# ai-forever/Kandinsky-2

Hardware: NVIDIA H100
Metric: unet_denoising_steps_per_sec (higher is better)
Workload: dtype f16

## Files before the change

include/k2b200.h:

```cpp
#ifndef K2B200_H_
#define K2B200_H_

#include <stdint.h>

#ifdef __cplusplus
extern "C" {
#endif

typedef void* k2_stream_t;

const char* k2_last_error(void);
int k2_version(void);
long long k2_launch_count(void);
void k2_reset_launch_count(void);
int k2_set_tuning(int key, int value);

typedef struct {
  const void* ptr;
  int C;
  int ld;
  int taps;
} K2ConvSrc;

int k2_conv_gemm(const K2ConvSrc* srcs, int nsrc, int NB, int H, int W, const void* w_packed, int w_rows,
                 int Ktot, int ldw, int Cout, const float* bias, const void* residual, int ldr, void* out, int ldo,
                 int out_mode, void* workspace, long long workspace_bytes, float* gn_partial, int* info,
                 k2_stream_t stream);

int k2_conv_gemm_cfg(const K2ConvSrc* srcs, int nsrc, int NB, int H, int W, const void* w_packed, int w_rows,
                     int Ktot, int ldw, int Cout, const float* bias, const void* residual, int ldr, void* out, int ldo,
                     int out_mode, void* workspace, long long workspace_bytes, float* gn_partial, int* info,
                     const int* cfg, long long w_batch_stride, k2_stream_t stream);

int k2_conv_plan(int NB, int H, int W, int taps, int Ktot, int Cout, int out_mode, long long workspace_bytes,
                 int want_gn_partial, int* info);

long long k2_gn_scratch_floats(int NB, int HW, int C);
int k2_gn_stats(const void* src0, int C0, int ld0, const void* src1, int C1, int ld1, int NB, int HW,
                int groups, float eps, float* stats, float* scratch, k2_stream_t stream);
int k2_gn_finalize(const float* part0, int C0, int rg0, const float* part1, int C1, int rg1, int NB, int HW, int groups,
                   float eps, float* stats, k2_stream_t stream);
int k2_gn_apply(const void* src0, int C0, int ld0, const void* src1, int C1, int ld1, int NB, int H, int W,
                int groups, const float* stats, const float* gamma, const float* beta, const float* film,
                int film_ld, int act, int resample, void* y, int ldy, void* xres, int ldx, const float* zq, int zh,
                int zw, const float* sn_w, k2_stream_t stream);
int k2_gn_apply_fold(const void* src0, int C0, int ld0, const void* src1, int C1, int ld1, int NB, int H, int W, int groups,
                     const float* part0, int rg0, const float* part1, int rg1, float eps, const float* gamma,
                     const float* beta, const float* film, int film_ld, int act, int resample, void* y, int ldy, void* xres,
                     int ldx, k2_stream_t stream);

int k2_attention_d64(const void* qkv, int ldq, int hs, int q_off, int k_off, int v_off, const void* enc,
                     int lde, int ehs, int ek_off, int ev_off, int B, int heads, int T, int Tc, float scale,
                     void* out, int ldo, k2_stream_t stream);

int k2_attention_d512(const void* qkv, int ldq, int q_off, int k_off, int v_off, int B, int T, float scale, void* out, int ldo,
                      k2_stream_t stream);

int k2_linear(const float* x, int ldx, const void* W, int w_is_half, const float* b, const float* add,
              int ldadd, float* y, int ldy, int M, int N, int K, int silu_in, int silu_out,
              k2_stream_t stream);
int k2_layernorm(const float* x, const float* gamma, const float* beta, float* y, int M, int N, float eps,
                 k2_stream_t stream);
int k2_timestep_embedding(const float* t, float* out, int B, int dim, float max_period, k2_stream_t stream);
int k2_f32_to_f16(const float* x, void* y, long long n, k2_stream_t stream);
int k2_silu_f16(const void* x, void* y, long long n, k2_stream_t stream);

int k2_stem_im2col(const float* x, int Cx, const float* x2, int C2, const float* x3, int C3, int mul23,
                   int NB, int H, int W, void* out, int Kpad, k2_stream_t stream);
// ... 92 lines not shown
```

kandinsky-2_b200/csrc/k2_api.cu:

```cuda
#include <stdio.h>
#include <stdlib.h>
#include <string.h>

#include <algorithm>
#include <atomic>
#include <mutex>

#include "../../include/k2b200.h"
#include "k2_internal.h"

namespace k2 {

static thread_local std::string g_err;
static std::atomic<long long> g_launches{0};
static int g_force_bn = 0;
static int g_force_split = 0;
static int g_pdl = 0;


void set_error(const std::string& msg) { g_err = msg; }
int fail(const std::string& msg) {
  g_err = msg;
  return -1;
}
void count_launch(int n) { g_launches.fetch_add(n, std::memory_order_relaxed); }

bool pdl_enabled() { return g_pdl != 0; }
static int g_gn_bps = 0;
int gn_apply_blocks_per_sm() { return g_gn_bps; }

int num_sms() {
  static int n = 0;
  if (n == 0) {
    int dev = 0;
    cudaGetDevice(&dev);
    cudaDeviceGetAttribute(&n, cudaDevAttrMultiProcessorCount, dev);
    if (n <= 0) n = 132;
  }
  return n;
}

typedef CUresult (*EncodeTiledFn)(CUtensorMap*, CUtensorMapDataType, cuuint32_t, void*, const cuuint64_t*,
                                  const cuuint64_t*, const cuuint32_t*, const cuuint32_t*,
                                  CUtensorMapInterleave, CUtensorMapSwizzle, CUtensorMapL2promotion,
                                  CUtensorMapFloatOOBfill);

static EncodeTiledFn get_encode_fn() {
  static EncodeTiledFn fn = nullptr;
  static std::once_flag once;
  std::call_once(once, [] {
// ... 49 lines not shown
      const long long tiles = tiles_h * tiles_w * ((NB + tn - 1) / tn);
      for (int k = (tn == 1 ? 0 : 1); k < 2; ++k) {
        bool better = best_tiles[k] < 0 || tiles < best_tiles[k];
        if (!better && tiles == best_tiles[k]) {
          if (tn != bn[k]) {
            better = tn < bn[k];
          } else {
            const int d_new = tw > th ? tw - th : th - tw;
            const int d_old = bw[k] > bh[k] ? bw[k] - bh[k] : bh[k] - bw[k];
            better = (d_new < d_old) || (d_new == d_old && tw > bw[k]);
          }
        }
        if (better) {
          best_tiles[k] = tiles;
          bn[k] = tn;
          bw[k] = tw;
          bh[k] = th;
        }
      }
    }
  }
  const int k = (!single_image_only && best_tiles[1] * 100 <= best_tiles[0] * 85) ? 1 : 0;
  TN = bn[k];
  TW = bw[k];
  TH = bh[k];
}


struct ConvPlan {
  int TN, TH, TW, tiles_w, tiles_h, tiles_n, m_tiles;
  int m_tiles_phase;
  int BN, splits;
  int fuse_stats, row_groups;
};

static void plan_conv(int NB, int H, int W, bool any9, int kchunks, int Cout, int out_mode, bool has_workspace,
                      long long workspace_bytes, bool want_gn, ConvPlan& pl, const int* cfg = nullptr, bool up2 = false,
                      bool w_batched = false) {
  const int g_force_bn = (cfg && cfg[0]) ? cfg[0] : k2::g_force_bn;
  const int g_force_split = (cfg && cfg[2]) ? cfg[2] : k2::g_force_split;
  choose_tile(NB, H, W, pl.TN, pl.TH, pl.TW, w_batched);
  pl.tiles_w = (W + pl.TW - 1) / pl.TW;
  pl.tiles_h = (H + pl.TH - 1) / pl.TH;
  pl.tiles_n = (NB + pl.TN - 1) / pl.TN;
  pl.m_tiles = pl.tiles_w * pl.tiles_h * pl.tiles_n;
  pl.m_tiles_phase = pl.m_tiles;

  int BN = g_force_bn;
  int splits = 1;
  const long long M_total = static_cast<long long>(NB) * H * W;
  const bool can_split = !up2 && !w_batched && has_workspace && out_mode == 0 && Cout % 8 == 0;
  auto split_ok = [&](int sp) {
    if (sp == 1) return true;
    const int kps = (kchunks + sp - 1) / sp;
    return can_split && kps >= 8 && (sp - 1) * kps < kchunks &&
           static_cast<long long>(sp) * M_total * Cout * 4 <= workspace_bytes;
  };
  auto model = [&](int bn, int sp) {
    const long long nt = (Cout + bn - 1) / bn;
    const long long units = static_cast<long long>(pl.m_tiles) * nt * sp * (up2 ? 4 : 1);
    const long long slots = num_sms();
    const long long waves = (units + slots - 1) / slots;
    const long long kps = (kchunks + sp - 1) / sp;
    long long cost = waves * (kps * (4LL * bn + 60) + 2000);
    if (sp > 1) cost += 4000 + (static_cast<long long>(sp) + 1) * M_total * Cout * 4 / 1800;
    return cost;
  };
  if (BN == 0) {
    if (Cout <= 16) BN = 16;
    else if (Cout <= 64) BN = 64;
    else if (Cout <= 128) BN = 128;
    else BN = 0;
  }
  {
    const int cand[3] = {256, 192, 128};
    long long best = -1;
    int best_bn = BN ? BN : 256, best_sp = 1;
    for (int ci = 0; ci < 3; ++ci) {
      const int bn = BN ? BN : cand[ci];
      if (BN && ci > 0) break;
      for (int sp = 1; sp <= 8; ++sp) {
        if (g_force_split > 0 && sp != g_force_split) continue;
        if (!split_ok(sp)) continue;
        const long long c = model(bn, sp);
        if (best < 0 || c < best) {
          best = c;
          best_bn = bn;
          best_sp = sp;
        }
      }
    }
    BN = best_bn;
    splits = best_sp;
  }
  pl.BN = BN;
  pl.splits = splits;

  pl.fuse_stats = 0;
  pl.row_groups = 0;
  if (want_gn && out_mode == 0 && Cout % 8 == 0) {
    if (splits == 1 && BN >= 64 && Cout % 64 == 0 && (pl.TN == 1 || pl.TH * pl.TW == 16)) {
      pl.fuse_stats = 1;
      pl.row_groups = ((pl.TN == 1) ? pl.m_tiles : NB * pl.tiles_h * pl.tiles_w) * (up2 ? 4 : 1);
    } else if (splits > 1 && (static_cast<long long>(H) * W) % 16 == 0) {
      pl.fuse_stats = 2;
      pl.row_groups = static_cast<int>(M_total / 16);
    }
  }
}

static void plan_to_info(const ConvPlan& pl, int* info) {
  if (!info) return;
  info[0] = pl.BN; info[1] = 0;
  info[2] = pl.splits; info[3] = pl.m_tiles; info[4] = pl.TN;
  info[5] = pl.fuse_stats; info[6] = pl.row_groups;
}

}

using namespace k2;

extern "C" {

const char* k2_last_error(void) { return g_err.c_str(); }
int k2_version(void) { return 100; }
long long k2_launch_count(void) { return g_launches.load(); }
void k2_reset_launch_count(void) { g_launches.store(0); }
int k2_set_tuning(int key, int value) {
  if (key == 0) {
    g_force_bn = value;
    return 0;
  }
  if (key == 1) {
    g_force_split = value;
    return 0;
  }
  if (key == 2) {
    if (value == 2) return fail("k2_set_tuning: no CTA-pair conv kernel on sm_90");
    return 0;
  }
  if (key == 4) {
    g_pdl = value;
    return 0;
  }
  if (key == 10) {
    return 0;
  }
  if (key == 11) {
    g_gn_bps = value;
    return 0;
  }
  if (key == 9) {
    return 0;
  }

  return fail("k2_set_tuning: unknown key");
}

int k2_conv_gemm(const K2ConvSrc* srcs, int nsrc, int NB, int H, int W, const void* w_packed, int w_rows,
                 int Ktot, int ldw, int Cout, const float* bias, const void* residual, int ldr, void* out, int ldo,
                 int out_mode, void* workspace, long long workspace_bytes, float* gn_partial, int* info,
                 k2_stream_t stream) {
  return k2_conv_gemm_cfg(srcs, nsrc, NB, H, W, w_packed, w_rows, Ktot, ldw, Cout, bias, residual, ldr, out, ldo, out_mode,
                          workspace, workspace_bytes, gn_partial, info, nullptr, 0, stream);
}

int k2_conv_gemm_cfg(const K2ConvSrc* srcs, int nsrc, int NB, int H, int W, const void* w_packed, int w_rows,
                     int Ktot, int ldw, int Cout, const float* bias, const void* residual, int ldr, void* out, int ldo,
                     int out_mode, void* workspace, long long workspace_bytes, float* gn_partial, int* info,
                     const int* cfg, long long w_batch_stride, k2_stream_t stream) {
  K2_REQUIRE(w_batch_stride >= 0 && w_batch_stride % 8 == 0, "conv_gemm_cfg: w_batch_stride must be a multiple of 8 elements");
  K2_REQUIRE(out_mode == 0 || out_mode == 1, "conv_gemm: out_mode must be 0 (fp16 rows) or 1 (fp32 NCHW)");
  K2_REQUIRE(out_mode == 0 || residual == nullptr, "conv_gemm: out_mode 1 (fp32 NCHW) takes no residual");
  const bool w_batched = w_batch_stride > 0;
  if (cfg) {
    K2_REQUIRE(cfg[0] == 0 || cfg[0] == 16 || cfg[0] == 64 || cfg[0] == 128 || cfg[0] == 192 || cfg[0] == 256,
               "conv_gemm_cfg: N tile must be 0, 16, 64, 128, 192 or 256");
    K2_REQUIRE(cfg[1] >= 0 && cfg[1] <= 2 && cfg[2] >= 0 && cfg[2] <= 8 && cfg[3] >= 0 && cfg[3] <= 2,
// ... 56 lines not shown
  p.up2 = up2 ? 1 : 0;
  p.a_box_bytes = static_cast<uint32_t>(p.TN * p.TH * p.TW * 128);
  for (int s = 0; s < nsrc; ++s) {
    const K2ConvSrc& src = srcs[s];
    uint64_t dims[4] = {static_cast<uint64_t>(src.C), static_cast<uint64_t>(W), static_cast<uint64_t>(H),
                        static_cast<uint64_t>(NB)};
    uint64_t str[3] = {static_cast<uint64_t>(src.ld) * 2, static_cast<uint64_t>(src.ld) * 2 * W,
                       static_cast<uint64_t>(src.ld) * 2 * W * H};
    uint32_t box[4] = {64, static_cast<uint32_t>(p.TW), static_cast<uint32_t>(p.TH), static_cast<uint32_t>(p.TN)};
    if (encode_tmap_f16(&p.tmA[s], src.ptr, 4, dims, str, box)) return -1;
  }
  const int BN = pl.BN, splits = pl.splits, fuse_stats = pl.fuse_stats;
  p.splits = splits;
  p.k_per_split = (kchunks + splits - 1) / splits;
  p.M_total = static_cast<long long>(NB) * H * W * (up2 ? 4 : 1);
  p.ws = reinterpret_cast<float*>(workspace);
  p.n_tiles = (Cout + BN - 1) / BN;
  p.Cout = Cout;
  {
    uint64_t dims[3] = {static_cast<uint64_t>(Ktot), static_cast<uint64_t>(w_rows), static_cast<uint64_t>(w_batched ? NB : 1)};
    uint64_t str[2] = {static_cast<uint64_t>(ldw) * 2,
                       (w_batched ? static_cast<uint64_t>(w_batch_stride) : static_cast<uint64_t>(ldw) * w_rows) * 2};
    uint32_t box[3] = {64, static_cast<uint32_t>(BN), 1};
    if (encode_tmap_f16(&p.tmB, w_packed, 3, dims, str, box)) return -1;
  }
  p.bias = bias;
  p.residual = reinterpret_cast<const __half*>(residual);
  p.ldr = ldr;
  p.out = out;
  p.ldo = ldo;
  p.out_mode = (splits > 1) ? 2 : out_mode;
  p.gn_part = (fuse_stats == 1) ? reinterpret_cast<float2*>(gn_partial) : nullptr;
  p.gn_mode = (fuse_stats == 1) ? (p.TN == 1 ? 1 : 2) : 0;
  if (out_mode == 0) {
    K2_REQUIRE(ldo % 8 == 0 && (reinterpret_cast<uintptr_t>(out) & 15) == 0, "conv_gemm: out alignment");
    if (residual)
      K2_REQUIRE(ldr % 8 == 0 && (reinterpret_cast<uintptr_t>(residual) & 15) == 0, "conv_gemm: residual alignment");
  }
  int rc = launch_conv_gemm(p, BN, static_cast<cudaStream_t>(stream));
  if (rc == 0) g_launches.fetch_add(1, std::memory_order_relaxed);
  if (rc == 0 && splits > 1) {
    rc = launch_splitk_finalize(p.ws, splits, p.M_total, Cout, bias, p.residual, ldr, reinterpret_cast<__half*>(out), ldo,
                                fuse_stats == 2 ? reinterpret_cast<float2*>(gn_partial) : nullptr,
                                static_cast<cudaStream_t>(stream));
    if (rc == 0) g_launches.fetch_add(1, std::memory_order_relaxed);
  }
  return rc;
}

int k2_conv_plan(int NB, int H, int W, int taps, int Ktot, int Cout, int out_mode, long long workspace_bytes,
                 int want_gn_partial, int* info) {
  K2_REQUIRE(NB > 0 && H > 0 && W > 0 && Cout > 0 && info, "conv_plan: bad arguments");
  K2_REQUIRE(Ktot > 0 && Ktot % 64 == 0, "conv_plan: Ktot must be a positive multiple of 64");
  ConvPlan pl;
  plan_conv(NB, H, W, taps == 9, Ktot / 64, Cout, out_mode, workspace_bytes > 0, workspace_bytes, want_gn_partial != 0, pl);
  plan_to_info(pl, info);
  return 0;
}

}
```

kandinsky-2_b200/csrc/k2_conv_gemm.cu:

```cuda
#include <stdio.h>

#include "k2_common.cuh"
#include "k2_internal.h"

namespace k2 {

namespace {

constexpr int BM = 128;
constexpr int BK = 64;
constexpr int A_STAGE_BYTES = BM * BK * 2;
constexpr int EPI_WARP_BYTES = 16 * 128;
constexpr int SMEM_LIMIT = 227 * 1024;

template <int BN>
struct Cfg {
  static constexpr int B_STAGE_BYTES = BN * BK * 2;
  static constexpr int STAGE_BYTES = A_STAGE_BYTES + B_STAGE_BYTES;
  static constexpr int EPI_BYTES = 8 * (EPI_WARP_BYTES + BN * 4);
  static constexpr int BAR_BYTES = 256;
  static constexpr int FIXED = EPI_BYTES + BAR_BYTES + 1024;
  static constexpr int STAGES = (SMEM_LIMIT - FIXED) / STAGE_BYTES > 6 ? 6 : (SMEM_LIMIT - FIXED) / STAGE_BYTES;
  static constexpr int SMEM_BYTES = STAGES * STAGE_BYTES + FIXED;
  static_assert(STAGES >= 2, "conv_gemm: shared memory does not hold two pipeline stages");
};

__device__ __forceinline__ void decode_m_tile(const ConvGemmParams& p, int m_idx, int& n0, int& y0,
                                              int& x0, int& phase) {
  phase = 0;
  if (p.up2) {
    phase = m_idx / p.m_tiles_phase;
    m_idx -= phase * p.m_tiles_phase;
  }
  int tw_i = m_idx % p.tiles_w;
  int t = m_idx / p.tiles_w;
  int th_i = t % p.tiles_h;
  int tn_i = t / p.tiles_h;
  x0 = tw_i * p.TW;
  y0 = th_i * p.TH;
  n0 = tn_i * p.TN;
}

__device__ __forceinline__ void ldsm_x4(uint32_t (&r)[4], uint32_t saddr) {
  asm volatile("ldmatrix.sync.aligned.m8n8.x4.shared.b16 {%0, %1, %2, %3}, [%4];"
               : "=r"(r[0]), "=r"(r[1]), "=r"(r[2]), "=r"(r[3])
               : "r"(saddr)
               : "memory");
}

template <int BN>
__device__ __forceinline__ void epilogue_warp(const ConvGemmParams& p, const float (&acc)[BN / 2], float* epi, uint32_t stg,
                                              const float* bsm, int k, int lane, int n0, int y0, int x0, int cbase, int split,
                                              int m_idx, int phase) {
  const int thw = p.TH * p.TW;
  auto out_row_of = [&](int row, int& n, int& y, int& x) -> long long {
    const int tn = row / thw;
    const int rem = row - tn * thw;
    const int th = rem / p.TW;
    const int tw = rem - th * p.TW;
    n = n0 + tn;
    y = y0 + th;
    x = x0 + tw;
    if (tn >= p.TN || n >= p.NB || y >= p.H || x >= p.W) return -1;
    return p.up2 ? (static_cast<long long>(n) * (2 * p.H) + (2 * y + (phase >> 1))) * (2 * p.W) + (2 * x + (phase & 1))
                 : (static_cast<long long>(n) * p.H + y) * p.W + x;
  };
  const int t4 = lane & 3, ra = lane >> 2;
  if constexpr (BN % 64 == 0) {
    if ((p.out_mode == 0 && p.Cout % 64 == 0) || (p.out_mode == 2 && p.Cout % 32 == 0)) {
      int n_, y_, x_;
      const int my_pix = static_cast<int>(out_row_of(16 * k + (lane & 15), n_, y_, x_));
      const int sub = lane >> 3, piece = lane & 7;
      int pix[4];
// ... 142 lines not shown
      return;
    }
  }
  int n[2], y[2], x[2];
  long long orow[2];
#pragma unroll
  for (int h = 0; h < 2; ++h) orow[h] = out_row_of(16 * k + ra + 8 * h, n[h], y[h], x[h]);
#pragma unroll
  for (int q = 0; q < BN / 8; ++q) {
#pragma unroll
    for (int h = 0; h < 2; ++h) {
#pragma unroll
      for (int e = 0; e < 2; ++e) {
        const int col = cbase + 8 * q + 2 * t4 + e;
        if (orow[h] < 0 || col >= p.Cout) continue;
        float f = acc[4 * q + 2 * h + e];
        if (p.out_mode == 2) {
          p.ws[(static_cast<long long>(split) * p.M_total + orow[h]) * p.Cout + col] = f;
          continue;
        }
        if (p.bias) f += __ldg(p.bias + col);
        if (p.out_mode == 0) {
          if (p.residual) f += __half2float(p.residual[orow[h] * p.ldr + col]);
          reinterpret_cast<__half*>(p.out)[orow[h] * p.ldo + col] = __float2half_rn(f);
        } else {
          reinterpret_cast<float*>(p.out)[((static_cast<long long>(n[h]) * p.Cout + col) * p.H + y[h]) * p.W + x[h]] = f;
        }
      }
    }
  }
}


template <int BN>
__global__ void __launch_bounds__(384, 1) conv_gemm_kernel(const __grid_constant__ ConvGemmParams p) {
  using C = Cfg<BN>;
  constexpr int NA = BN / 2;
  extern __shared__ uint8_t smem_raw[];
  uint8_t* smem = reinterpret_cast<uint8_t*>((reinterpret_cast<uintptr_t>(smem_raw) + 1023) &
                                             ~static_cast<uintptr_t>(1023));
  float* epi = reinterpret_cast<float*>(smem + C::STAGES * C::STAGE_BYTES);
  uint64_t* full_bar = reinterpret_cast<uint64_t*>(smem + C::STAGES * C::STAGE_BYTES + C::EPI_BYTES);
  uint64_t* empty_bar = full_bar + C::STAGES;

  const int warp_idx = threadIdx.x >> 5;
  const int lane = threadIdx.x & 31;
  const int wg = warp_idx >> 2;

  if (threadIdx.x == 0) {
    tma_prefetch_desc(&p.tmB);
    for (int s = 0; s < 3; ++s)
      if (p.seg_taps[s]) tma_prefetch_desc(&p.tmA[s]);
    for (int i = 0; i < C::STAGES; ++i) {
      mbar_init(&full_bar[i], 1);
      mbar_init(&empty_bar[i], 8);
    }
    fence_barrier_init();
  }
  __syncthreads();
  pdl_wait();
  pdl_launch();

  const int total_tiles = p.m_tiles * p.n_tiles * p.splits;

  if (wg == 0) {
    setmaxnreg_dec<40>();
    if (warp_idx == 0 && elect_one()) {
      int stage = 0;
      uint32_t ring_phase = 0;
      const uint32_t tx_bytes = p.a_box_bytes + C::B_STAGE_BYTES;
      for (int tile = blockIdx.x; tile < total_tiles; tile += gridDim.x) {
        const int n_idx = tile % p.n_tiles;
        const int m_idx = (tile / p.n_tiles) % p.m_tiles;
        const int split = tile / (p.m_tiles * p.n_tiles);
        int n0, y0, x0, phase;
        decode_m_tile(p, m_idx, n0, y0, x0, phase);
        const int kb = phase * p.num_k_chunks;
        const int k0 = split * p.k_per_split;
        const int k1 = min(p.num_k_chunks, k0 + p.k_per_split);
        int s = 0, rem = k0;
        while (rem >= p.seg_taps[s] * p.seg_kchunks[s]) {
          rem -= p.seg_taps[s] * p.seg_kchunks[s];
          ++s;
        }
        int tap = rem / p.seg_kchunks[s];
        int c = rem - tap * p.seg_kchunks[s];
        for (int kc = k0; kc < k1; ++kc) {
          const int taps = p.seg_taps[s];
          const int dy = (taps == 9) ? (tap / 3 - 1) : (taps == 4 ? (tap >> 1) + (phase >> 1) - 1 : 0);
          const int dx = (taps == 9) ? (tap % 3 - 1) : (taps == 4 ? (tap & 1) + (phase & 1) - 1 : 0);
          mbar_wait_lean(&empty_bar[stage], ring_phase ^ 1);
          uint8_t* sA = smem + stage * C::STAGE_BYTES;
          uint8_t* sB = sA + A_STAGE_BYTES;
          mbar_arrive_expect_tx(&full_bar[stage], tx_bytes);
          tma_load_4d(sA, &p.tmA[s], &full_bar[stage], c * BK, x0 + dx, y0 + dy, n0);
          tma_load_3d(sB, &p.tmB, &full_bar[stage], (kb + kc) * BK, n_idx * BN, p.w_batched ? n0 : 0);
          if (++stage == C::STAGES) {
            stage = 0;
            ring_phase ^= 1;
          }
          if (++c == p.seg_kchunks[s]) {
            c = 0;
            if (++tap == taps) {
              tap = 0;
              ++s;
            }
          }
        }
      }
    }
  } else {
    setmaxnreg_inc<232>();
    const int g = wg - 1;
    const int k = warp_idx - 4;
    const uint32_t stg = smem_u32(epi) + k * EPI_WARP_BYTES;
    float* bsm = epi + 8 * EPI_WARP_BYTES / 4 + k * BN;
    int bias_cols = -1;
    int stage = 0;
    uint32_t phase = 0;
    for (int tile = blockIdx.x; tile < total_tiles; tile += gridDim.x) {
      const int n_idx = tile % p.n_tiles;
      const int m_idx = (tile / p.n_tiles) % p.m_tiles;
      const int split = tile / (p.m_tiles * p.n_tiles);
      const int nk = min(p.num_k_chunks, (split + 1) * p.k_per_split) - split * p.k_per_split;
      float acc[NA];
#pragma unroll
      for (int i = 0; i < NA; ++i) acc[i] = 0.f;
      int prev_stage = -1;
      for (int kc = 0; kc < nk; ++kc) {
        mbar_wait_lean(&full_bar[stage], phase);
        const uint32_t a_addr = smem_u32(smem + stage * C::STAGE_BYTES) + g * (64 * 128);
        const uint32_t b_addr = smem_u32(smem + stage * C::STAGE_BYTES + A_STAGE_BYTES);
        wgmma_fence();
#pragma unroll
        for (int ks = 0; ks < BK / 16; ++ks) {
          const uint64_t adesc = make_wgmma_desc(a_addr) + static_cast<uint64_t>(ks * 2);
          const uint64_t bdesc = make_wgmma_desc(b_addr) + static_cast<uint64_t>(ks * 2);
          if constexpr (BN == 256) {
            wgmma_m64n256k16(acc, adesc, bdesc, 1u);
          } else if constexpr (BN == 192) {
            wgmma_m64n192k16(acc, adesc, bdesc, 1u);
          } else if constexpr (BN == 128) {
            wgmma_m64n128k16(acc, adesc, bdesc, 1u);
          } else if constexpr (BN == 64) {
            wgmma_m64n64k16(acc, adesc, bdesc, 1u);
          } else {
            static_assert(BN == 16, "conv_gemm: N tile without a wgmma shape");
            wgmma_m64n16k16(acc, adesc, bdesc, 1u);
          }
        }
        wgmma_commit();
        wgmma_wait<1>();
        if (prev_stage >= 0 && lane == 0) mbar_arrive(&empty_bar[prev_stage]);
        prev_stage = stage;
        if (++stage == C::STAGES) {
          stage = 0;
          phase ^= 1;
        }
      }
      wgmma_wait<0>();
#pragma unroll
      for (int i = 0; i < NA; ++i) reg_fence(acc[i]);
      if (prev_stage >= 0 && lane == 0) mbar_arrive(&empty_bar[prev_stage]);

      int n0, y0, x0, mphase;
      decode_m_tile(p, m_idx, n0, y0, x0, mphase);
      const int cbase = n_idx * BN;
      if (p.bias && cbase != bias_cols) {
        __syncwarp();
#pragma unroll
        for (int c = lane; c < BN; c += 32) bsm[c] = (cbase + c < p.Cout) ? __ldg(p.bias + cbase + c) : 0.f;
        __syncwarp();
        bias_cols = cbase;
      }
      epilogue_warp<BN>(p, acc, epi, stg, bsm, k, lane, n0, y0, x0, cbase, split, m_idx, mphase);
    }
  }
}

__global__ void __launch_bounds__(256) splitk_finalize_kernel(const float* __restrict__ ws, int splits, long long M,
                                                              int Cout, const float* __restrict__ bias,
                                                              const __half* __restrict__ residual, int ldr,
                                                              __half* __restrict__ out, int ldo, float2* __restrict__ gn_part) {
  __shared__ float red[8][32][17];
  const int vx = threadIdx.x & 31, ry = threadIdx.x >> 5;
  const int c0 = (blockIdx.y * 32 + vx) * 8;
  const long long rg = blockIdx.x;
  pdl_wait();
  pdl_launch();
  float st[16];
#pragma unroll
  for (int e = 0; e < 16; ++e) st[e] = 0.f;
  if (c0 < Cout) {
    float bv[8];
#pragma unroll
    for (int e = 0; e < 8; ++e) bv[e] = bias ? __ldg(bias + c0 + e) : 0.f;
#pragma unroll
// ... 25 lines not shown
        oh[e] = __floats2half2_rn(f[2 * e], f[2 * e + 1]);
        const float2 t = __half22float2(oh[e]);
        st[2 * e] += t.x;
        st[2 * e + 1] += t.y;
        st[8 + 2 * e] = fmaf(t.x, t.x, st[8 + 2 * e]);
        st[8 + 2 * e + 1] = fmaf(t.y, t.y, st[8 + 2 * e + 1]);
      }
      *reinterpret_cast<uint4*>(out + m * ldo + c0) = ov;
    }
  }
  if (gn_part == nullptr) return;
#pragma unroll
  for (int e = 0; e < 16; ++e) red[ry][vx][e] = st[e];
  __syncthreads();
  const int vx2 = threadIdx.x >> 3, e2 = threadIdx.x & 7;
  const int c = (blockIdx.y * 32 + vx2) * 8 + e2;
  if (c < Cout) {
    float s1 = 0.f, s2 = 0.f;
#pragma unroll
    for (int q = 0; q < 8; ++q) {
      s1 += red[q][vx2][e2];
      s2 += red[q][vx2][8 + e2];
    }
    gn_part[rg * Cout + c] = make_float2(s1, s2);
  }
}


template <int BN>
int launch_bn(const ConvGemmParams& p, cudaStream_t stream) {
  using C = Cfg<BN>;
  static bool attr_set = false;
  if (!attr_set) {
    K2_CHECK_CUDA(cudaFuncSetAttribute(conv_gemm_kernel<BN>, cudaFuncAttributeMaxDynamicSharedMemorySize, C::SMEM_BYTES));
    attr_set = true;
  }
  int total = p.m_tiles * p.n_tiles * p.splits;
  int grid = total < num_sms() ? total : num_sms();
  K2_CHECK_CUDA(launch_k(conv_gemm_kernel<BN>, dim3(grid), dim3(384), C::SMEM_BYTES, stream, p));
  return 0;
}

}

int launch_splitk_finalize(const float* ws, int splits, long long M, int Cout, const float* bias, const __half* residual,
                           int ldr, __half* out, int ldo, float2* gn_part, cudaStream_t stream) {
  dim3 grid(static_cast<unsigned int>((M + 15) / 16), (Cout / 8 + 31) / 32);
  K2_CHECK_CUDA(launch_k(splitk_finalize_kernel, grid, dim3(256), 0, stream, ws, splits, M, Cout, bias, residual, ldr, out, ldo,
                         gn_part));
  return 0;
}

int launch_conv_gemm(const ConvGemmParams& p, int BN, cudaStream_t stream) {
  switch (BN) {
    case 16: return launch_bn<16>(p, stream);
    case 64: return launch_bn<64>(p, stream);
    case 128: return launch_bn<128>(p, stream);
    case 192: return launch_bn<192>(p, stream);
    case 256: return launch_bn<256>(p, stream);
    default: return fail("conv_gemm: unsupported BN");
  }
}

}
```

kandinsky-2_b200/csrc/k2_internal.h:

```cpp
#pragma once
#include <cuda.h>
#include <cuda_fp16.h>
#include <cuda_runtime.h>
#include <stdint.h>

#include <string>

namespace k2 {

void set_error(const std::string& msg);
int fail(const std::string& msg);
#define K2_CHECK_CUDA(expr)                                                                 \
  do {                                                                                      \
    cudaError_t _e = (expr);                                                                \
    if (_e != cudaSuccess)                                                                  \
      return ::k2::fail(std::string(#expr) + ": " + cudaGetErrorString(_e));                \
  } while (0)
#define K2_REQUIRE(cond, msg)                                  \
  do {                                                         \
    if (!(cond)) return ::k2::fail(std::string("k2b200: ") + (msg)); \
  } while (0)

inline bool aligned16(const void* p) { return (reinterpret_cast<uintptr_t>(p) & 15) == 0; }

// ... 17 lines not shown
}
void count_launch(int n = 1);

int encode_tmap_f16(CUtensorMap* out, const void* base, int rank, const uint64_t* dims,
                    const uint64_t* strides_bytes , const uint32_t* box);

struct ConvGemmParams {
  CUtensorMap tmA[3];
  CUtensorMap tmB;
  int w_batched;
  int seg_taps[3];
  int seg_kchunks[3];
  int num_k_chunks;
  int NB, H, W;
  int TN, TH, TW;
  int tiles_n, tiles_h, tiles_w;
  int m_tiles, n_tiles;
  int Cout;
  const float* bias;
  const __half* residual;
  int ldr;
  void* out;
  int ldo;
  int out_mode;
  uint32_t a_box_bytes;
  int splits;
  int k_per_split;
  float* ws;
  long long M_total;
  float2* gn_part;
  int gn_mode;
  int up2;
  int m_tiles_phase;
};
int launch_conv_gemm(const ConvGemmParams& p, int BN, cudaStream_t stream);
int launch_splitk_finalize(const float* ws, int splits, long long M, int Cout, const float* bias, const __half* residual,
                           int ldr, __half* out, int ldo, float2* gn_part, cudaStream_t stream);

struct FlashParams {
  const __half* qkv;
  long long ldq;
  int hs, q_off, k_off, v_off;
  const __half* enc;
  long long lde;
  int ehs, ek_off, ev_off;
  int B, heads, T, Tc;
  __half* out;
  int ldo, ohs;
  float scale_log2e;
};
int gn_apply_blocks_per_sm();
int launch_attention(const FlashParams& p, int head_dim, cudaStream_t stream);

}
```

kandinsky-2_b200/kandinsky2/_native.py:

```python
import ctypes
import os

_HERE = os.path.dirname(os.path.abspath(__file__))
LIB_PATH = os.path.join(os.path.dirname(_HERE), "libk2b200.so")

_lib = None
MISSING = []


class K2Error(RuntimeError):
    pass


class K2ConvSrc(ctypes.Structure):
    _fields_ = [("ptr", ctypes.c_void_p), ("C", ctypes.c_int), ("ld", ctypes.c_int), ("taps", ctypes.c_int)]


_P = ctypes.c_void_p
_I = ctypes.c_int
_F = ctypes.c_float
_LL = ctypes.c_longlong

SIGNATURES = {
    "k2_last_error": (ctypes.c_char_p, []),
    "k2_version": (_I, []),
    "k2_launch_count": (_LL, []),
    "k2_reset_launch_count": (None, []),
    "k2_set_tuning": (_I, [_I, _I]),
    "k2_conv_gemm": (_I, [ctypes.POINTER(K2ConvSrc), _I, _I, _I, _I, _P, _I, _I, _I, _I, _P, _P, _I, _P, _I, _I, _P, _LL, _P,
                         ctypes.POINTER(ctypes.c_int), _P]),
    "k2_conv_gemm_cfg": (_I, [ctypes.POINTER(K2ConvSrc), _I, _I, _I, _I, _P, _I, _I, _I, _I, _P, _P, _I, _P, _I, _I, _P, _LL, _P,
                             ctypes.POINTER(ctypes.c_int), ctypes.POINTER(ctypes.c_int), _LL, _P]),
    "k2_sn_apply": (_I, [_P, _I, _I, _I, _I, _I, _I, _P, _P, _P, _P, _I, _I, _P, _I, _P, _I, _P]),
    "k2_transpose_f16": (_I, [_P, _I, _P, _I, _I, _I, _P]),
    "k2_gn_finalize": (_I, [_P, _I, _I, _P, _I, _I, _I, _I, _I, _F, _P, _P]),
    "k2_upsample2x_nhwc": (_I, [_P, _I, _P, _I, _I, _I, _I, _I, _P]),
    "k2_subsample2_nhwc": (_I, [_P, _I, _P, _I, _I, _I, _I, _I, _I, _I, _P]),
    "k2_softmax_rows": (_I, [_P, _I, _P, _I, _LL, _I, _F, _P]),
    "k2_layernorm_f16": (_I, [_P, _I, _P, _P, _P, _I, _I, _I, _F, _P]),
    "k2_gelu_f16": (_I, [_P, _P, _LL, _P]),
    "k2_quick_gelu_f16": (_I, [_P, _P, _LL, _P]),
    "k2_attention_small": (_I, [_P, _I, _P, _I, _P, _I, _I, _I, _I, _F, _P]),
    "k2_prior_tokens": (_I, [_P, _I, _P, _I, _P, _I, _I, _I, _P]),
    "k2_f16_to_f32": (_I, [_P, _I, _P, _I, _I, _I, _P]),
    "k2_clip_patchify": (_I, [_P, _I, _I, _I, _P, _I, _I, _P]),
    "k2_attention_heads": (_I, [_P, _I, _I, _I, _I, _I, _I, _I, _I, _I, _F, _P, _I, _I, _P]),
    "k2_clip_text_embed": (_I, [_P, _I, _I, _I, _P, _I, _P, _I, _P, _I, _P]),
    "k2_clip_text_pool": (_I, [_P, _I, _I, _I, _I, _P, _I, _I, _P, _I, _P, _P]),
    "k2_xlmr_embed": (_I, [_P, _I, _I, _I, _I, _P, _I, _P, _I, _P, _P, _P, _F, _P, _I, _I, _P]),
    "k2_masked_mean_f16": (_I, [_P, _I, _P, _I, _I, _I, _I, _P, _I, _P]),
    "k2_conv_plan": (_I, [_I, _I, _I, _I, _I, _I, _I, _LL, _I, _P]),
    "k2_gn_scratch_floats": (_LL, [_I, _I, _I]),
    "k2_gn_stats": (_I, [_P, _I, _I, _P, _I, _I, _I, _I, _I, _F, _P, _P, _P]),
    "k2_gn_apply": (_I, [_P, _I, _I, _P, _I, _I, _I, _I, _I, _I, _P, _P, _P, _P, _I, _I, _I, _P, _I, _P, _I, _P,
                         _I, _I, _P, _P]),
    "k2_gn_apply_fold": (_I, [_P, _I, _I, _P, _I, _I, _I, _I, _I, _I, _P, _I, _P, _I, _F, _P, _P, _P, _I, _I, _I, _P, _I, _P,
                              _I, _P]),
    "k2_attention_d64": (_I, [_P, _I, _I, _I, _I, _I, _P, _I, _I, _I, _I, _I, _I, _I, _I, _F, _P, _I, _P]),
    "k2_attention_d512": (_I, [_P, _I, _I, _I, _I, _I, _I, _F, _P, _I, _P]),
    "k2_linear": (_I, [_P, _I, _P, _I, _P, _P, _I, _P, _I, _I, _I, _I, _I, _I, _P]),
    "k2_layernorm": (_I, [_P, _P, _P, _P, _I, _I, _F, _P]),
    "k2_timestep_embedding": (_I, [_P, _P, _I, _I, _F, _P]),
    "k2_f32_to_f16": (_I, [_P, _P, _LL, _P]),
    "k2_silu_f16": (_I, [_P, _P, _LL, _P]),
    "k2_stem_im2col": (_I, [_P, _I, _P, _I, _P, _I, _I, _I, _I, _I, _P, _I, _P]),
    "k2_sampler_step": (_I, [_P, _P, _P, _P, _I, _I, _I, _F, _I, _F, _I, _P, _P, _P, _P, _P]),
    "k2_step_begin": (_I, [_P, _P, _LL, _P, _I, _P, _P, _P, _P, _P, _P, _P]),
    "k2_step_end": (_I, [_P, _P]),
    "k2_plms_step": (_I, [_P, _I, _P, _P, _P, _P, _P, _P, _P, _I, _I, _I, _F, _I, _P]),
    "k2_dpm_solver_step": (_I, [_P, _I, _P, _P, _P, _I, _I, _I, _F, _I, _P, _P, _P, _P]),
    "k2_dpm_solver_sde_step": (_I, [_P, _I, _P, _P, _P, _P, _I, _I, _I, _F, _I, _P, _P, _P, _P]),
    "k2_unipc_step": (_I, [_P, _I, _P, _P, _P, _P, _P, _P, _I, _I, _I, _F, _I, _P, _P, _P, _P]),
    "k2_heun_step": (_I, [_P, _I, _P, _P, _P, _P, _I, _I, _I, _F, _I, _P, _P, _P, _P]),
    "k2_vq_argmin": (_I, [_P, _P, _P, _I, _I, _I, _P]),
    "k2_pointwise_nchw_f32": (_I, [_P, _P, _P, _P, _I, _I, _I, _I, _P]),
    "k2_nchw_to_nhwc_f32": (_I, [_P, _P, _I, _I, _I, _I, _P]),
    "k2_images_to_u8": (_I, [_P, _P, _I, _I, _I, _I, _I, _I, _P]),
    "k2_lora_merge": (_I, [_P, _I, _P, _P, _I, _I, _I, _F, _P, _I, _P]),
    "k2_relu_f16": (_I, [_P, _I, _P, _I, _I, _I, _P]),
    "k2_relu_f32": (_I, [_P, _I, _P, _I, _I, _I, _P]),
    "k2_bilinear_f16": (_I, [_P, _I, _I, _I, _I, _I, _P, _I, _I, _I, _I, _P]),
    "k2_depth_to_space_f16": (_I, [_P, _I, _I, _I, _I, _I, _I, _P, _I, _P]),
    "k2_readout_rows_f16": (_I, [_P, _I, _I, _I, _I, _P, _I, _P]),
    "k2_im2col_f16": (_I, [_P, _I, _I, _I, _I, _I, _I, _I, _I, _I, _I, _P, _I, _I, _P]),
# ... 41 lines not shown
```

kandinsky-2_b200/kandinsky2/ops.py:

```python
import ctypes

import torch

from . import _native as nat
from ._native import K2ConvSrc, check, ptr, stream_ptr


def _row_stride(t):
    assert t.stride(-1) == 1, "channel dim must be contiguous"
    ld = t.stride(-2)
    n = t.shape[-2]
    for d in range(t.dim() - 3, -1, -1):
        assert t.shape[d] == 1 or t.stride(d) == ld * n, f"not a row-strided NHWC view: {t.shape} {t.stride()}"
        n *= t.shape[d]
    return ld


def _pad64(c):
    return (c + 63) // 64 * 64


def pack_conv_weight(w, split=None):
    w = w.detach()
    if w.dim() == 2:
# ... 63 lines not shown
    arr = (K2ConvSrc * len(srcs))()
    for i, (t, taps) in enumerate(srcs):
        assert t.dtype == torch.float16 and t.is_cuda
        arr[i].ptr = t.data_ptr()
        arr[i].C = t.shape[-1]
        arr[i].ld = _row_stride(t)
        arr[i].taps = taps
    if out is None:
        if out_mode == 0:
            out = torch.empty((NB, H, W, cout), dtype=torch.float16, device=t0.device)
        else:
            out = torch.empty((NB, cout, H, W), dtype=torch.float32, device=t0.device)
    ldo = _row_stride(out) if out_mode == 0 else 0
    ldr = _row_stride(residual) if residual is not None else 0
    assert w_packed.dtype == torch.float16 and w_packed.stride(1) == 1
    ws = _workspace(t0.device)
    _info = (ctypes.c_int * 7)()
    _cfg = (ctypes.c_int * 4)(*cfg) if cfg is not None else None
    check(lib.k2_conv_gemm_cfg(arr, len(srcs), NB, H, W, ptr(w_packed), w_packed.shape[0], w_packed.shape[1],
                               w_packed.stride(0), cout,
                               ptr(bias), ptr(residual), ldr, ptr(out), ldo, out_mode, ptr(ws), ws.numel(), ptr(gn_part),
                               _info, _cfg, int(w_batch_stride), stream_ptr()))
    if info is not None:
        info[:] = list(_info)
    return out


def conv_plan(NB, H, W, taps, ktot, cout, out_mode=0, workspace_bytes=_CONV_WS_BYTES, want_gn_partial=True):
    lib = nat.load()
    info = (ctypes.c_int * 7)()
    check(lib.k2_conv_plan(NB, H, W, taps, ktot, cout, out_mode, workspace_bytes, int(want_gn_partial), info))
    keys = ("n_tile", "cta_pair", "splits", "m_tiles", "images_per_tile", "gn_partial_mode", "row_groups")
    return dict(zip(keys, list(info)))


def gemm_rows(x, w_packed, cout, bias=None, residual=None, out=None, cfg=None, info=None):
    lead = x.shape[:-1]
    M = 1
    for d in lead:
        M *= d
    x3 = x.reshape(1, 1, M, x.shape[-1]) if x.is_contiguous() else None
    if x3 is None:
        x3 = x.as_strided((1, 1, M, x.shape[-1]), (0, 0, x.stride(-2), 1))
    if out is None:
        out = torch.empty(tuple(lead) + (cout,), dtype=torch.float16, device=x.device)
    o3 = out.as_strided((1, 1, M, cout), (0, 0, out.stride(-2), 1))
    r3 = None
    if residual is not None:
        r3 = residual.as_strided((1, 1, M, cout), (0, 0, residual.stride(-2), 1))
    conv_gemm([(x3, 1)], w_packed, cout, bias=bias, residual=r3, out=o3, geom=(1, 1, M), cfg=cfg, info=info)
    return out


_gn_scratch = {}


_GN_SCRATCH_FLOATS = 1 << 23


def _scratch(dev, nfloats):
    key = (dev.index, )
    buf = _gn_scratch.get(key)
    if buf is None:
        buf = torch.zeros(_GN_SCRATCH_FLOATS, dtype=torch.float32, device=dev)
        _gn_scratch[key] = buf
    if nfloats > buf.numel():
# ... 624 lines not shown
```

Baseline: 32.83.

## Balance conv GEMM last wave with stream-K style tail splitting across CTAs

Adds a tail mode to the persistent conv GEMM kernel. The tiles left over after the last full wave are split along K evenly across all SMs, and partial accumulators are handed between neighbouring CTAs through workspace slots using acquire/release flags. The goal is to reduce wave quantization idle time when the tile count is not a multiple of the SM count. It adds a ticket-based CTA ordering, spin-waits between CTAs and extra fp32 workspace traffic, and is enabled automatically by a cost model.

```diff
diff --git a/include/k2b200.h b/include/k2b200.h
--- a/include/k2b200.h
+++ b/include/k2b200.h
@@ -34,6 +34,9 @@
 
 int k2_conv_plan(int NB, int H, int W, int taps, int Ktot, int Cout, int out_mode, long long workspace_bytes,
                  int want_gn_partial, int* info);
+
+int k2_conv_tail_plan(int NB, int H, int W, int taps, int Ktot, int Cout, int out_mode, long long workspace_bytes,
+                      int want_gn_partial, const int* cfg, int w_batched, int* tail, int* ranges);
 
 long long k2_gn_scratch_floats(int NB, int HW, int C);
 int k2_gn_stats(const void* src0, int C0, int ld0, const void* src1, int C1, int ld1, int NB, int HW,
diff --git a/kandinsky-2_b200/csrc/k2_api.cu b/kandinsky-2_b200/csrc/k2_api.cu
--- a/kandinsky-2_b200/csrc/k2_api.cu
+++ b/kandinsky-2_b200/csrc/k2_api.cu
@@ -16,6 +16,7 @@
 static int g_force_bn = 0;
 static int g_force_split = 0;
 static int g_pdl = 0;
+static int g_tail = 0;
 
 
 void set_error(const std::string& msg) { g_err = msg; }
@@ -131,6 +132,8 @@
   int m_tiles_phase;
   int BN, splits;
   int fuse_stats, row_groups;
+  int tail_first, tail_tiles;
+  int nk;
 };
 
 static void plan_conv(int NB, int H, int W, bool any9, int kchunks, int Cout, int out_mode, bool has_workspace,
@@ -195,6 +198,28 @@
   pl.BN = BN;
   pl.splits = splits;
 
+  pl.tail_first = 0;
+  pl.tail_tiles = 0;
+  pl.nk = kchunks;
+  {
+    const long long slots = num_sms();
+    const long long units = static_cast<long long>(pl.m_tiles) * ((Cout + BN - 1) / BN) * (up2 ? 4 : 1);
+    const long long scratch = slots * 128 * BN * 4;
+    if (g_tail != 1 && splits == 1 && BN <= TAIL_MAX_BN && !w_batched && slots <= TAIL_MAX_RANGES && units > slots &&
+        units % slots != 0 && has_workspace && scratch <= workspace_bytes) {
+      const long long F = units / slots, T = units - (F - 1) * slots;
+      const long long chunk = 4LL * BN + 60, unit = kchunks * chunk + 2000;
+      const long long whole = 2 * unit;
+      const long long tail = (T * kchunks + slots - 1) / slots * chunk + 2 * 2000 + 2 * scratch / 3000;
+      const long long waves = (units + slots - 1) / slots;
+      const bool sparse = 10 * units <= 9 * waves * slots;
+      if ((tail < whole && sparse) || g_tail == 2) {
+        pl.tail_first = static_cast<int>((F - 1) * slots);
+        pl.tail_tiles = static_cast<int>(T);
+      }
+    }
+  }
+
   pl.fuse_stats = 0;
   pl.row_groups = 0;
   if (want_gn && out_mode == 0 && Cout % 8 == 0) {
@@ -243,6 +268,11 @@
     return 0;
   }
   if (key == 10) {
+    return 0;
+  }
+  if (key == 12) {
+    K2_REQUIRE(value >= 0 && value <= 2, "k2_set_tuning: key 12 takes 0 (auto), 1 (off) or 2 (on)");
+    g_tail = value;
     return 0;
   }
   if (key == 11) {
@@ -365,6 +395,8 @@
   p.out_mode = (splits > 1) ? 2 : out_mode;
   p.gn_part = (fuse_stats == 1) ? reinterpret_cast<float2*>(gn_partial) : nullptr;
   p.gn_mode = (fuse_stats == 1) ? (p.TN == 1 ? 1 : 2) : 0;
+  p.tail_first = pl.tail_tiles ? pl.tail_first : p.m_tiles * p.n_tiles * splits;
+  p.tail_acc = pl.tail_tiles ? reinterpret_cast<float*>(workspace) : nullptr;
   if (out_mode == 0) {
     K2_REQUIRE(ldo % 8 == 0 && (reinterpret_cast<uintptr_t>(out) & 15) == 0, "conv_gemm: out alignment");
     if (residual)
@@ -391,4 +423,36 @@
   return 0;
 }
 
-}
+int k2_conv_tail_plan(int NB, int H, int W, int taps, int Ktot, int Cout, int out_mode, long long workspace_bytes,
+                      int want_gn_partial, const int* cfg, int w_batched, int* tail, int* ranges) {
+  K2_REQUIRE(NB > 0 && H > 0 && W > 0 && Cout > 0 && tail, "conv_tail_plan: bad arguments");
+  K2_REQUIRE(taps == 9 || taps == 1 || taps == 4, "conv_tail_plan: taps must be 9, 1 or 4");
+  const int kq = taps == 4 ? 4 * 64 : 64;
+  K2_REQUIRE(Ktot > 0 && Ktot % kq == 0, "conv_tail_plan: Ktot must be a positive multiple of 64 (of 256 for taps == 4)");
+  K2_REQUIRE(taps != 4 || (H % 2 == 0 && W % 2 == 0 && w_batched == 0), "conv_tail_plan: taps == 4 needs even H, W");
+  if (cfg)
+    K2_REQUIRE(cfg[0] == 0 || cfg[0] == 16 || cfg[0] == 64 || cfg[0] == 128 || cfg[0] == 192 || cfg[0] == 256,
+               "conv_tail_plan: N tile must be 0, 16, 64, 128, 192 or 256");
+  const bool up2 = taps == 4;
+  ConvPlan pl;
+  plan_conv(NB, up2 ? H / 2 : H, up2 ? W / 2 : W, taps != 1, Ktot / kq, Cout, out_mode, workspace_bytes > 0,
+            workspace_bytes, want_gn_partial != 0, pl, cfg, up2, w_batched != 0);
+  const int R = pl.tail_tiles ? num_sms() : 0;
+  tail[0] = R;
+  tail[1] = pl.tail_first;
+  tail[2] = pl.tail_tiles;
+  tail[3] = pl.nk;
+  tail[4] = pl.m_tiles * ((Cout + pl.BN - 1) / pl.BN) * pl.splits * (up2 ? 4 : 1);
+  tail[5] = pl.BN;
+  if (ranges) {
+    for (int r = 0; r < R; ++r) {
+      const TailRange t = tail_range(pl.tail_tiles, pl.nk, R, r);
+      int* o = ranges + 6 * r;
+      o[0] = t.lead_tile; o[1] = t.lead_end; o[2] = t.whole_begin; o[3] = t.whole_end; o[4] = t.trail_tile;
+      o[5] = t.trail_begin;
+    }
+  }
+  return 0;
+}
+
+}
diff --git a/kandinsky-2_b200/csrc/k2_conv_gemm.cu b/kandinsky-2_b200/csrc/k2_conv_gemm.cu
--- a/kandinsky-2_b200/csrc/k2_conv_gemm.cu
+++ b/kandinsky-2_b200/csrc/k2_conv_gemm.cu
@@ -39,6 +39,67 @@
   x0 = tw_i * p.TW;
   y0 = th_i * p.TH;
   n0 = tn_i * p.TN;
+}
+
+__device__ unsigned int g_tail_ticket;
+__device__ unsigned int g_tail_flag[TAIL_MAX_RANGES];
+
+__device__ __forceinline__ unsigned int ld_acquire_gpu(const unsigned int* p) {
+  unsigned int v;
+  asm volatile("ld.acquire.gpu.global.u32 %0, [%1];" : "=r"(v) : "l"(p) : "memory");
+  return v;
+}
+__device__ __forceinline__ void st_release_gpu(unsigned int* p, unsigned int v) {
+  asm volatile("st.release.gpu.global.u32 [%0], %1;" ::"l"(p), "r"(v) : "memory");
+}
+
+struct WorkItem {
+  int tile, k0, k1;
+  int kind;
+};
+struct WorkList {
+  int cta, n_head, n_tail;
+  WorkItem tail[4];
+  __device__ void build(const ConvGemmParams& p, int cta_, int total) {
+    cta = cta_;
+    n_head = cta < p.tail_first ? (p.tail_first - 1 - cta) / static_cast<int>(gridDim.x) + 1 : 0;
+    n_tail = 0;
+    if (p.tail_first == total) return;
+    const int t0 = p.tail_first, nk = p.num_k_chunks;
+    const TailRange tr = tail_range(total - t0, nk, gridDim.x, cta);
+    if (tr.lead_tile >= 0) tail[n_tail++] = WorkItem{t0 + tr.lead_tile, 0, tr.lead_end, 1};
+    for (int t = tr.whole_begin; t < tr.whole_end; ++t) tail[n_tail++] = WorkItem{t0 + t, 0, nk, 0};
+    if (tr.trail_tile >= 0) tail[n_tail++] = WorkItem{t0 + tr.trail_tile, tr.trail_begin, nk, 2};
+  }
+  __device__ __forceinline__ bool get(const ConvGemmParams& p, int it, WorkItem& w) const {
+    if (it < n_head) {
+      w.tile = cta + it * static_cast<int>(gridDim.x);
+      const int split = w.tile / (p.m_tiles * p.n_tiles);
+      w.k0 = split * p.k_per_split;
+      w.k1 = min(p.num_k_chunks, w.k0 + p.k_per_split);
+      w.kind = 0;
+      return true;
+    }
+    it -= n_head;
+    if (it >= n_tail) return false;
+    w = tail[it];
+    return true;
+  }
+};
+
+template <bool TAIL>
+__device__ __forceinline__ bool work_item(const ConvGemmParams& p, const WorkList& work, int it, WorkItem& w) {
+  if constexpr (TAIL) {
+    return work.get(p, it, w);
+  } else {
+    w.tile = blockIdx.x + it * gridDim.x;
+    if (w.tile >= p.m_tiles * p.n_tiles * p.splits) return false;
+    const int split = w.tile / (p.m_tiles * p.n_tiles);
+    w.k0 = split * p.k_per_split;
+    w.k1 = min(p.num_k_chunks, w.k0 + p.k_per_split);
+    w.kind = 0;
+    return true;
+  }
 }
 
 __device__ __forceinline__ void ldsm_x4(uint32_t (&r)[4], uint32_t saddr) {
@@ -247,7 +308,7 @@
 }
 
 
-template <int BN>
+template <int BN, bool TAIL>
 __global__ void __launch_bounds__(384, 1) conv_gemm_kernel(const __grid_constant__ ConvGemmParams p) {
   using C = Cfg<BN>;
   constexpr int NA = BN / 2;
@@ -276,7 +337,18 @@
   pdl_wait();
   pdl_launch();
 
-  const int total_tiles = p.m_tiles * p.n_tiles * p.splits;
+  WorkList& work = *reinterpret_cast<WorkList*>(smem + C::STAGES * C::STAGE_BYTES + C::EPI_BYTES + 128);
+  if (TAIL && threadIdx.x == 0) {
+    const int total_tiles = p.m_tiles * p.n_tiles * p.splits;
+    int cta = blockIdx.x;
+    {
+      const unsigned int t = atomicAdd(&g_tail_ticket, 1u);
+      if (t == gridDim.x - 1) atomicExch(&g_tail_ticket, 0u);
+      cta = static_cast<int>(t);
+    }
+    work.build(p, cta, total_tiles);
+  }
+  if constexpr (TAIL) __syncthreads();
 
   if (wg == 0) {
     setmaxnreg_dec<40>();
@@ -284,15 +356,14 @@
       int stage = 0;
       uint32_t ring_phase = 0;
       const uint32_t tx_bytes = p.a_box_bytes + C::B_STAGE_BYTES;
-      for (int tile = blockIdx.x; tile < total_tiles; tile += gridDim.x) {
-        const int n_idx = tile % p.n_tiles;
-        const int m_idx = (tile / p.n_tiles) % p.m_tiles;
-        const int split = tile / (p.m_tiles * p.n_tiles);
+      WorkItem w;
+      for (int it = 0; work_item<TAIL>(p, work, it, w); ++it) {
+        const int n_idx = w.tile % p.n_tiles;
+        const int m_idx = (w.tile / p.n_tiles) % p.m_tiles;
         int n0, y0, x0, phase;
         decode_m_tile(p, m_idx, n0, y0, x0, phase);
         const int kb = phase * p.num_k_chunks;
-        const int k0 = split * p.k_per_split;
-        const int k1 = min(p.num_k_chunks, k0 + p.k_per_split);
+        const int k0 = w.k0, k1 = w.k1;
         int s = 0, rem = k0;
         while (rem >= p.seg_taps[s] * p.seg_kchunks[s]) {
           rem -= p.seg_taps[s] * p.seg_kchunks[s];
@@ -333,14 +404,31 @@
     int bias_cols = -1;
     int stage = 0;
     uint32_t phase = 0;
-    for (int tile = blockIdx.x; tile < total_tiles; tile += gridDim.x) {
-      const int n_idx = tile % p.n_tiles;
-      const int m_idx = (tile / p.n_tiles) % p.m_tiles;
-      const int split = tile / (p.m_tiles * p.n_tiles);
-      const int nk = min(p.num_k_chunks, (split + 1) * p.k_per_split) - split * p.k_per_split;
+    const int ct = threadIdx.x - 128;
+    WorkItem w;
+    for (int it = 0; work_item<TAIL>(p, work, it, w); ++it) {
+      const int nk = w.k1 - w.k0;
       float acc[NA];
-#pragma unroll
-      for (int i = 0; i < NA; ++i) acc[i] = 0.f;
+      if (w.kind == 2) {
+        if (ct == 0) {
+          while (ld_acquire_gpu(&g_tail_flag[work.cta - 1]) == 0) {
+          }
+          g_tail_flag[work.cta - 1] = 0;
+        }
+        named_bar_sync(2, 256);
+      }
+      {
+        const float4* slot = reinterpret_cast<const float4*>(p.tail_acc) + static_cast<long long>(work.cta - 1) * (BM * BN / 4);
+#pragma unroll
+        for (int i = 0; i < NA / 4; ++i) {
+          float4 v = make_float4(0.f, 0.f, 0.f, 0.f);
+          if (w.kind == 2) v = __ldcg(slot + i * 256 + ct);
+          acc[4 * i] = v.x;
+          acc[4 * i + 1] = v.y;
+          acc[4 * i + 2] = v.z;
+          acc[4 * i + 3] = v.w;
+        }
+      }
       int prev_stage = -1;
       for (int kc = 0; kc < nk; ++kc) {
         mbar_wait_lean(&full_bar[stage], phase);
@@ -377,7 +465,21 @@
 #pragma unroll
       for (int i = 0; i < NA; ++i) reg_fence(acc[i]);
       if (prev_stage >= 0 && lane == 0) mbar_arrive(&empty_bar[prev_stage]);
-
+      work_item<TAIL>(p, work, it, w);
+      if (w.kind == 1) {
+        float4* slot = reinterpret_cast<float4*>(p.tail_acc) + static_cast<long long>(work.cta) * (BM * BN / 4);
+#pragma unroll
+        for (int i = 0; i < NA / 4; ++i)
+          __stcg(slot + i * 256 + ct, make_float4(acc[4 * i], acc[4 * i + 1], acc[4 * i + 2], acc[4 * i + 3]));
+        __threadfence();
+        named_bar_sync(2, 256);
+        if (ct == 0) st_release_gpu(&g_tail_flag[work.cta], 1u);
+        continue;
+      }
+
+      const int n_idx = w.tile % p.n_tiles;
+      const int m_idx = (w.tile / p.n_tiles) % p.m_tiles;
+      const int split = w.tile / (p.m_tiles * p.n_tiles);
       int n0, y0, x0, mphase;
       decode_m_tile(p, m_idx, n0, y0, x0, mphase);
       const int cbase = n_idx * BN;
@@ -469,12 +571,20 @@
   using C = Cfg<BN>;
   static bool attr_set = false;
   if (!attr_set) {
-    K2_CHECK_CUDA(cudaFuncSetAttribute(conv_gemm_kernel<BN>, cudaFuncAttributeMaxDynamicSharedMemorySize, C::SMEM_BYTES));
+    K2_CHECK_CUDA(cudaFuncSetAttribute(conv_gemm_kernel<BN, false>, cudaFuncAttributeMaxDynamicSharedMemorySize, C::SMEM_BYTES));
+    if constexpr (BN <= TAIL_MAX_BN)
+      K2_CHECK_CUDA(cudaFuncSetAttribute(conv_gemm_kernel<BN, true>, cudaFuncAttributeMaxDynamicSharedMemorySize, C::SMEM_BYTES));
     attr_set = true;
   }
   int total = p.m_tiles * p.n_tiles * p.splits;
   int grid = total < num_sms() ? total : num_sms();
-  K2_CHECK_CUDA(launch_k(conv_gemm_kernel<BN>, dim3(grid), dim3(384), C::SMEM_BYTES, stream, p));
+  if constexpr (BN <= TAIL_MAX_BN) {
+    if (p.tail_first < total) {
+      K2_CHECK_CUDA(launch_k(conv_gemm_kernel<BN, true>, dim3(grid), dim3(384), C::SMEM_BYTES, stream, p));
+      return 0;
+    }
+  }
+  K2_CHECK_CUDA(launch_k(conv_gemm_kernel<BN, false>, dim3(grid), dim3(384), C::SMEM_BYTES, stream, p));
   return 0;
 }
 
diff --git a/kandinsky-2_b200/csrc/k2_internal.h b/kandinsky-2_b200/csrc/k2_internal.h
--- a/kandinsky-2_b200/csrc/k2_internal.h
+++ b/kandinsky-2_b200/csrc/k2_internal.h
@@ -73,7 +73,29 @@
   int gn_mode;
   int up2;
   int m_tiles_phase;
+  int tail_first;
+  float* tail_acc;
 };
+
+struct TailRange {
+  int lead_tile, lead_end, whole_begin, whole_end, trail_tile, trail_begin;
+};
+__host__ __device__ inline TailRange tail_range(int T, int nk, int R, int r) {
+  const long long L = static_cast<long long>(T) * nk;
+  const long long a = L * r / R, b = L * (r + 1) / R;
+  const int ta = static_cast<int>(a / nk), sa = static_cast<int>(a % nk);
+  const int tb = static_cast<int>(b / nk), eb = static_cast<int>(b % nk);
+  TailRange t;
+  t.trail_tile = sa ? ta : -1;
+  t.trail_begin = sa;
+  t.whole_begin = sa ? ta + 1 : ta;
+  t.whole_end = tb;
+  t.lead_tile = eb ? tb : -1;
+  t.lead_end = eb;
+  return t;
+}
+constexpr int TAIL_MAX_RANGES = 256;
+constexpr int TAIL_MAX_BN = 128;
 int launch_conv_gemm(const ConvGemmParams& p, int BN, cudaStream_t stream);
 int launch_splitk_finalize(const float* ws, int splits, long long M, int Cout, const float* bias, const __half* residual,
                            int ldr, __half* out, int ldo, float2* gn_part, cudaStream_t stream);
diff --git a/kandinsky-2_b200/kandinsky2/_native.py b/kandinsky-2_b200/kandinsky2/_native.py
--- a/kandinsky-2_b200/kandinsky2/_native.py
+++ b/kandinsky-2_b200/kandinsky2/_native.py
@@ -50,6 +50,7 @@
     "k2_xlmr_embed": (_I, [_P, _I, _I, _I, _I, _P, _I, _P, _I, _P, _P, _P, _F, _P, _I, _I, _P]),
     "k2_masked_mean_f16": (_I, [_P, _I, _P, _I, _I, _I, _I, _P, _I, _P]),
     "k2_conv_plan": (_I, [_I, _I, _I, _I, _I, _I, _I, _LL, _I, _P]),
+    "k2_conv_tail_plan": (_I, [_I, _I, _I, _I, _I, _I, _I, _LL, _I, _P, _I, _P, _P]),
     "k2_gn_scratch_floats": (_LL, [_I, _I, _I]),
     "k2_gn_stats": (_I, [_P, _I, _I, _P, _I, _I, _I, _I, _I, _F, _P, _P, _P]),
     "k2_gn_apply": (_I, [_P, _I, _I, _P, _I, _I, _I, _I, _I, _I, _P, _P, _P, _P, _I, _I, _I, _P, _I, _P, _I, _P,
diff --git a/kandinsky-2_b200/kandinsky2/ops.py b/kandinsky-2_b200/kandinsky2/ops.py
--- a/kandinsky-2_b200/kandinsky2/ops.py
+++ b/kandinsky-2_b200/kandinsky2/ops.py
@@ -119,6 +119,22 @@
     check(lib.k2_conv_plan(NB, H, W, taps, ktot, cout, out_mode, workspace_bytes, int(want_gn_partial), info))
     keys = ("n_tile", "cta_pair", "splits", "m_tiles", "images_per_tile", "gn_partial_mode", "row_groups")
     return dict(zip(keys, list(info)))
+
+
+def conv_tail_plan(NB, H, W, taps, ktot, cout, out_mode=0, workspace_bytes=_CONV_WS_BYTES, want_gn_partial=True, cfg=None,
+                   w_batched=False):
+    lib = nat.load()
+    tail = (ctypes.c_int * 6)()
+    _cfg = (ctypes.c_int * 4)(*cfg) if cfg is not None else None
+    args = (NB, H, W, taps, ktot, cout, out_mode, workspace_bytes, int(want_gn_partial), _cfg, int(w_batched))
+    check(lib.k2_conv_tail_plan(*args, tail, None))
+    R = tail[0]
+    rng = (ctypes.c_int * max(1, 6 * R))()
+    check(lib.k2_conv_tail_plan(*args, tail, rng))
+    keys = ("ranges", "first", "tiles", "nk", "units", "n_tile")
+    out = dict(zip(keys, list(tail)))
+    out["per_range"] = [tuple(rng[6 * r:6 * r + 6]) for r in range(R)]
+    return out
 
 
 def gemm_rows(x, w_packed, cout, bias=None, residual=None, out=None, cfg=None, info=None):
diff --git a/profiles/conv_tail.py b/profiles/conv_tail.py
--- /dev/null
+++ b/profiles/conv_tail.py
@@ -0,0 +1,85 @@
+import argparse
+import json
+import os
+import subprocess
+import sys
+
+ROOT = os.path.dirname(os.path.dirname(os.path.abspath(__file__)))
+sys.path[:0] = [ROOT, os.path.join(ROOT, "kandinsky-2_b200")]
+
+import torch
+
+LAYERS = [
+    ("96x96 384->384 3x3", 8, 96, 96, [(384, 9)], 384, 128, True),
+    ("48x48 768->768 3x3", 8, 48, 48, [(768, 9)], 768, 128, True),
+    ("48x48 768 3x3 + 1x1 skip [768 | 384]", 8, 48, 48, [(768, 9), (768, 1), (384, 1)], 768, 128, False),
+    ("48x48 384->768 3x3 + 1x1 skip", 8, 48, 48, [(384, 9), (384, 1)], 768, 128, False),
+    ("24x24 1152->1152 3x3", 8, 24, 24, [(1152, 9)], 1152, 128, True),
+    ("48x48 768 1x1 + res", 8, 48, 48, [(768, 1)], 768, 128, True),
+    ("gemm 1152x1536->4608", 1, 1, 1152, [(1536, 1)], 4608, 128, False),
+    ("96x96 384->8 3x3 fp32 head", 8, 96, 96, [(384, 9)], 8, 16, False),
+]
+
+
+def _time(fn, min_ms=30.0, windows=5):
+    fn()
+    torch.cuda.synchronize()
+    e0, e1 = torch.cuda.Event(enable_timing=True), torch.cuda.Event(enable_timing=True)
+    e0.record()
+    fn()
+    e1.record()
+    torch.cuda.synchronize()
+    reps = max(1, int(min_ms / max(e0.elapsed_time(e1), 1e-3)) + 1)
+    out = []
+    for _ in range(windows):
+        e0.record()
+        for _ in range(reps):
+            fn()
+        e1.record()
+        torch.cuda.synchronize()
+        out.append(e0.elapsed_time(e1) / reps)
+    return sorted(out)[windows // 2]
+
+
+def main():
+    ap = argparse.ArgumentParser()
+    ap.add_argument("--out", default=None)
+    args = ap.parse_args()
+    from kandinsky2 import ops
+    ops.set_tuning(4, 1)
+    g = torch.Generator(device="cuda").manual_seed(0)
+    smi = subprocess.run(["nvidia-smi", "--query-gpu=name,power.limit,clocks.max.sm", "--format=csv,noheader"],
+                         capture_output=True, text=True).stdout.strip()
+    rows = []
+    for name, NB, H, W, srcs_spec, cout, bn, res in LAYERS:
+        srcs = [((torch.randn(NB, H, W, c, device="cuda", generator=g)).half(), taps) for c, taps in srcs_spec]
+        ktot = sum(taps * ((c + 63) // 64) * 64 for c, taps in srcs_spec)
+        wp = ops.pad_rows((torch.randn(cout, ktot, device="cuda", generator=g) / ktot ** 0.5).half().contiguous(), bn)
+        out_mode = 1 if cout < 64 else 0
+        kw = dict(bias=torch.randn(cout, device="cuda", generator=g), out_mode=out_mode)
+        if res:
+            kw["residual"] = torch.randn(NB, H, W, cout, device="cuda", generator=g).half()
+        taps = 9 if any(t == 9 for _, t in srcs_spec) else 1
+        ops.set_tuning(12, 2)
+        plan = ops.conv_tail_plan(NB, H, W, taps, ktot, cout, out_mode=out_mode, cfg=(bn, 0, 1, 0))
+        run = lambda: ops.conv_gemm(srcs, wp, cout, cfg=(bn, 0, 1, 0), **kw)
+        t = {1: [], 2: []}
+        for _ in range(3):
+            for mode in (1, 2):
+                ops.set_tuning(12, mode)
+                t[mode].append(_time(run))
+        ops.set_tuning(12, 0)
+        off, on = sorted(t[1])[1], sorted(t[2])[1]
+        units = plan["units"]
+        row = dict(layer=name, n_tile=bn, units=units, tail_units=plan["tiles"], last_wave_fill=units / (132 * -(-units // 132)),
+                   off_us=off * 1e3, on_us=on * 1e3, gain=(off - on) / off)
+        rows.append(row)
+        print(f"{name:40s} N {bn:3d} units {units:5d} fill {row['last_wave_fill']:.3f}  off {off * 1e3:8.1f} us  "
+              f"on {on * 1e3:8.1f} us  gain {100 * row['gain']:+.1f} %", flush=True)
+    if args.out:
+        with open(args.out, "w") as f:
+            json.dump(dict(gpu=smi, layers=rows), f, indent=1)
+
+
+if __name__ == "__main__":
+    main()
```

Result: no change. 32.80 (median of 6 runs) (-0.1%).
